# althonos/pyfastani

Hardware: AMD Instinct MI355X
Metric: genome-pair ANI/sec (5 Mb bacterial, 3 kb frags) (higher is better)
Workload: dtype u32

## Files before the change

### pyfastani_amd/csrc/fa_map.hip.h

```cpp
#pragma once

#include "fa_common.h"
#include "fa_compact.hip.h"
#include "fa_mapstream.h"
#include "fa_policy.h"
#include "fa_sketch.hip.h"
#include "fa_sketch_fast.hip.h"

namespace fa {



constexpr int MAP_THREADS = 256;
constexpr uint32_t SEED_PAD = 0xFFFFFFFFu;

__device__ inline void block_bitonic_sort(uint32_t *a, uint32_t n32) {
  for (uint32_t size = 2; size <= n32; size <<= 1) {
    for (uint32_t stride = size >> 1; stride > 0; stride >>= 1) {
      __syncthreads();
      for (uint32_t t = threadIdx.x; t < n32 / 2; t += blockDim.x) {
        uint32_t lo = 2 * t - (t & (stride - 1));
        uint32_t hi = lo + stride;
        bool up = (lo & size) == 0;
        uint32_t x = a[lo], y = a[hi];
// ... 1441 lines not shown
    atomicAdd(&a.counters[CNT_OFF_FAST], 1u);
  }
  __threadfence_block();
  __syncthreads();
  const uint32_t nl = sh_cnt, base = sh_base;
  for (uint32_t q = tid; q < nl; q += NT) {
    const uint32_t li = base + q;
    a.l_frag[li] = f; a.l_rfirst[li] = S_rfirst[q]; a.l_rpart[li] = S_rpart[q]; a.l_rlast[li] = S_rlast[q];
  }
  l1_locus_fields<NT>(a.ix, len, nl, S_rfirst, S_rpart, S_rlast, a.l_seq + base, a.l_start + base, a.l_end + base);
  __threadfence_block();
  __syncthreads();
  if (wv == 0) l1_number_groups(a.ix, nl, a.l_seq + base, a.l_group + base, base);
}

struct TieKey {
  uint32_t flip, add;
  __host__ __device__ uint32_t encode(uint32_t x) const { return (x + add) ^ flip; }
  __host__ __device__ uint32_t decode(uint32_t low) const { return (low ^ flip) - add; }
  static TieKey of(int largest) { TieKey t; t.flip = largest ? 0u : 0xFFFFFFFFu; t.add = largest ? 1u : 0u; return t; }
};

struct L2Args {
  IndexView ix;
  const uint32_t *q_hash;
  const int32_t *q_size;
  const int32_t *l_frag, *l_seq, *l_start, *l_end, *l_group, *l_rfirst, *l_rlast, *l_rpart;
  int32_t frag_len;
  int32_t *l_beg, *l_end0, *l_last;
  int32_t *l_ndrop;
  uint32_t *l_nev;
  uint32_t *l_ioff;
  unsigned long long *pinfo;
  uint64_t items_cap;
  int32_t l_cap;
  void *items;
  int32_t *l_shared, *l_pos;
  const int32_t *pass_lut;
  unsigned long long *group_best;
  const uint32_t *counters;
  LociRegions loci;
  int32_t qcap, cmw;
  int32_t cnt_slots;
  int32_t lanes;
  int32_t ev_stage;
  unsigned long long *rec_total;
  unsigned long long *ev_region, *rec_region;
  uint64_t region_cap;
  uint32_t n_regions;
  uint8_t *l_redo;
  uint32_t *redo_count;
  const uint32_t *f_loci_lo, *f_loci_n;
  const int32_t *frag_order;
  unsigned long long *stamp;
  uint32_t *scan_hist, *scan_cursor;
  uint32_t *scan_order;
  int32_t scan_class_div;
  int32_t slide_end;
  TieKey tie;
};

constexpr int L2_THREADS = 64;
constexpr int EV_THREADS = 256;
constexpr int SCAN_CLASSES = 32;
__device__ __forceinline__ uint32_t scan_class(uint32_t nev, int32_t div) {
  return (uint32_t)(SCAN_CLASSES - 1) - min((uint32_t)(SCAN_CLASSES - 1), nev / (uint32_t)div);
}

template <typename T> struct EvBits;
template <> struct EvBits<uint16_t> { static constexpr int RANK = EV_RANK16; };
template <> struct EvBits<uint32_t> { static constexpr int RANK = 24; };
constexpr int EV_DM = 0, EV_DW = 2, EV_DROP = 5, EV_SLOT = 6;
template <typename T> constexpr uint32_t ev_noeval() { return 1u << (8 * sizeof(T) - 1); }
template <typename T> constexpr uint32_t ev_slot_mask() { return ((1u << EvBits<T>::RANK) - 1u) << EV_SLOT; }
static_assert(EV_SLOT + EvBits<uint16_t>::RANK == 15 && EV_SLOT + EvBits<uint32_t>::RANK <= 31, "event fields overlap");

#ifndef FA_EV_WAVES
#define FA_EV_WAVES 8
#endif
constexpr int EV_WAVES_PER_SIMD = FA_EV_WAVES;
constexpr int EV_SENTINELS = 4;
#ifndef FA_EV_RPL
#define FA_EV_RPL 4
#endif
constexpr int EV_RPL = FA_EV_RPL;
static_assert(EV_RPL >= 1 && EV_RPL <= 4, "the last trip of a phase is dispatched on 1..4 records per lane");
__host__ __device__ inline size_t ev_sketch_bytes(int cnt_slots) { return ((size_t)(cnt_slots - 1 + EV_SENTINELS) * 4 + 15) / 16 * 16; }

constexpr int EV_OCC_BITS = 10, EV_SUB_BITS = 5;
template <typename T, bool PACKED>
__global__ __launch_bounds__(EV_THREADS, EV_WAVES_PER_SIMD) void k_l2_events(L2Args a) {
  extern __shared__ __align__(16) unsigned char lds[];
  stage_stamp(a.stamp);
  uint32_t *Q = (uint32_t *)lds;
  constexpr int QT_BITS = EV_OCC_BITS + EV_SUB_BITS;
  constexpr int OCC_N = (1 << EV_OCC_BITS) + 1;
  constexpr uint32_t SUB_MASK = (1u << EV_SUB_BITS) - 1u;
  static_assert(EV_SUB_BITS == 5, "one 32-bit occupancy word per bucket");
  __shared__ __align__(8) unsigned char rank_table[OCC_N * 4 + (OCC_N + 1) * 2];
  uint32_t *const OCC = (uint32_t *)rank_table;
  uint16_t *const R0 = (uint16_t *)(rank_table + OCC_N * 4);
  const int f = a.frag_order ? a.frag_order[blockIdx.x] : (int)blockIdx.x;
  if (f < 0) return;
  const uint32_t l_lo = a.f_loci_lo[f], l_n = a.f_loci_n[f];
  if (l_n == 0) return;
  const int s = a.q_size[f];
  const int lane = threadIdx.x & 63, wv = threadIdx.x >> 6;
  if (a.counters[CNT_LOCI_OVF] || s > a.cnt_slots - 1) return;
  for (int i = threadIdx.x; i < s + EV_SENTINELS; i += EV_THREADS) Q[i] = i < s ? a.q_hash[(size_t)f * a.qcap + i] : 0xFFFFFFFFu;
  for (int b = threadIdx.x; b < OCC_N; b += EV_THREADS) { OCC[b] = 0u; R0[b] = (uint16_t)s; }
  __shared__ uint32_t sh_wave[EV_THREADS / 64];
  __shared__ uint32_t sh_run, sh_base, sh_ok;
  __shared__ unsigned long long sh_records;
  __shared__ uint32_t sh_class[SCAN_CLASSES];
  if (threadIdx.x == 0) { sh_run = 0; sh_records = 0; }
  if (threadIdx.x < SCAN_CLASSES) sh_class[threadIdx.x] = 0;
  __syncthreads();
  const int32_t *wpos = a.ix.rec_wpos;
  for (uint32_t c0 = 0; c0 < l_n; c0 += EV_THREADS) {
    const uint32_t l = l_lo + c0 + threadIdx.x;
    uint32_t nev = 0, records = 0;
    if (c0 + threadIdx.x < l_n) {
      const int lo = a.ix.contig_rec[a.l_seq[l]];
      const int rfirst = a.l_rfirst[l], target = a.l_start[l], rpart = a.l_rpart[l];
      int last = a.ix.rec_fwd[a.l_rlast[l]];
      if (a.slide_end) {
        const int tgt = wpos[a.l_rlast[l]] + a.frag_len;
        int u = last, v = min(a.ix.contig_rec[a.l_seq[l] + 1], last + (a.frag_len - a.cmw));
        while (u < v) { int mid = u + ((v - u) >> 1); if (wpos[mid] < tgt) u = mid + 1; else v = mid; }
        last = u;
      }
      int x = max(lo, rfirst - a.frag_len), y = rfirst;
      if (rpart >= 0) {
        y = min(rfirst, a.ix.rec_bwd[rpart] + 1);
        x = max(x, y - (a.frag_len - a.cmw + 1));
      }
      while (x < y) { int mid = x + ((y - x) >> 1); if (wpos[mid] < target) x = mid + 1; else y = mid; }
      const int beg = x;
      const int end0 = a.ix.rec_fwd[beg];
      const int ndrop = last > end0 ? a.ix.rec_bwd[last - 1] - beg : 0;
      a.l_beg[l] = beg; a.l_end0[l] = end0; a.l_last[l] = last; a.l_ndrop[l] = ndrop;
      nev = (uint32_t)((((end0 - beg + 7) & ~7) + (last - end0) + ndrop + 7) & ~7);
      records = (uint32_t)(last - beg);
      a.l_nev[l] = nev;
      if (a.scan_class_div) atomicAdd(&sh_class[scan_class(nev, a.scan_class_div)], 1u);
    }
    uint32_t incl = nev;
    for (int d = 1; d < 64; d <<= 1) { uint32_t o = __shfl_up(incl, d); if (lane >= d) incl += o; }
    if (lane == 63) sh_wave[wv] = incl;
    uint32_t rsum = records;
    for (int d = 32; d > 0; d >>= 1) rsum += __shfl_down(rsum, d);
    if (lane == 0) atomicAdd(&sh_records, (unsigned long long)rsum);
    __syncthreads();
    uint32_t off = sh_run + incl - nev;
    for (int q = 0; q < wv; q++) off += sh_wave[q];
// ... 175 lines not shown
        const int rem = hi - t0;
        auto tail = [&](auto rpl_tag) __attribute__((always_inline)) { issue(rpl_tag, t, FIRST, t0, hi); work(rpl_tag, first_tag, store, t, cur, t0, hi); };
        if (rem > 64 * 3) tail(std::integral_constant<int, (EV_RPL >= 4 ? 4 : EV_RPL)>());
        else if (rem > 64 * 2) tail(std::integral_constant<int, (EV_RPL >= 3 ? 3 : EV_RPL)>());
        else if (rem > 64) tail(std::integral_constant<int, (EV_RPL >= 2 ? 2 : EV_RPL)>());
        else if (rem > 0) tail(std::integral_constant<int, 1>());
      };
      phase(std::true_type(), cur.beg, cur.end0);
      phase(std::false_type(), cur.end0, cur.last);
    };
    if (st.staged) run([&](uint32_t pos, uint32_t v) __attribute__((always_inline)) { *(lds_out_t)(uintptr_t)(obase + pos * (uint32_t)sizeof(T)) = (T)v; });
    else { T *gout = st.gout; run([&](uint32_t pos, uint32_t v) __attribute__((always_inline)) { gout[pos] = (T)v; }); }
    end_locus(st);
  }
}

template <typename T, typename ST, int LNT, bool BASE0>
struct Slide {
  typedef __attribute__((address_space(3))) ST *lds_ptr;
  static constexpr int STB = (int)sizeof(ST);
  static constexpr int SBITS = 8 * STB;
  static constexpr int RB = EvBits<T>::RANK;
  int lbase, LNB, s;
  int rl, g, shared, best, beg, opt_s, opt_e;
  uint32_t overflow;

  static __device__ __forceinline__ uint32_t ld(int addr) { return (uint32_t)*(lds_ptr)(uintptr_t)(uint32_t)addr; }
  static __device__ __forceinline__ void sto(int addr, uint32_t v) { *(lds_ptr)(uintptr_t)(uint32_t)addr = (ST)v; }

  __device__ __forceinline__ void init(ST *st, int lane, int lanes, int sketch, int beg0) {
    lbase = (int)(uint32_t)(uintptr_t)(lds_ptr)st + lane * STB;
    LNB = (LNT ? LNT : lanes) * STB;
    s = sketch;
    rl = lbase; g = 0; shared = 0; best = -1; beg = opt_s = opt_e = beg0; overflow = 0;
  }
  static constexpr uint32_t EMPTY = 2u;
  __device__ __forceinline__ void clear() { for (int i = 0; i <= s + 1; i++) sto(i * LNB + lbase, EMPTY); }
  template <int SH> __device__ __forceinline__ int slot_addr(uint32_t word) const {
    if constexpr (LNT == 64) {
      const uint32_t row = (SH ? word >> SH : word) & ev_slot_mask<T>();
      if constexpr (BASE0) return (int)((STB == 1 ? row : row * STB) | (uint32_t)lbase);
      else return (int)(STB == 1 ? row : row * STB) + lbase;
    } else {
      return (int)__builtin_amdgcn_ubfe(word, SH + EV_SLOT, RB) * LNB + lbase;
    }
  }
  template <int SH> __device__ __forceinline__ void fill(uint32_t word) {
    const int dM = __builtin_amdgcn_sbfe(word, SH + EV_DM, 2), dW = __builtin_amdgcn_sbfe(word, SH + EV_DW, 2);
    const int addr = slot_addr<SH>(word);
    const uint32_t nv = (ld(addr) + (uint32_t)(dW << 1)) ^ ((uint32_t)dM & 1u);
    overflow |= nv;
    sto(addr, nv);
  }
  __device__ __forceinline__ void read_pivot() {
    int rstar = s, F = s, acc = 0, m_acc = 0;
    bool hit = false;
    for (int r = 0; r < s; r++) {
      const uint32_t v = ld((r + 1) * LNB + lbase);
      const int c = (int)(v >> 1) - 1, mt = (int)(v & 1u);
      const bool now = !hit && r + acc + c >= s;
      rstar = now ? r : rstar;
      F = now ? r + acc : F;
      shared = now ? m_acc : shared;
      hit = hit || now;
      acc += c; m_acc += mt;
    }
    F = hit ? F : s + acc;
    shared = hit ? shared : m_acc;
    g = F - s;
    rl = rstar * LNB + lbase;
    best = shared;
  }
  template <int SH> __device__ __forceinline__ void step(uint32_t word) {
    const int dM = __builtin_amdgcn_sbfe(word, SH + EV_DM, 2), dW = __builtin_amdgcn_sbfe(word, SH + EV_DW, 2);
    const int drp = (int)__builtin_amdgcn_ubfe(word, SH + EV_DROP, 1);
    const int addr = slot_addr<SH>(word);
    const int addrb = rl + drp * LNB;
    const uint32_t v = ld(addr), vb0 = ld(addrb);
    const uint32_t nv = (v + (uint32_t)(dW << 1)) ^ ((uint32_t)dM & 1u);
    overflow |= nv;
    sto(addr, nv);
    const bool below = addr <= rl;
    const int dWb = below ? dW : 0;
    shared += below ? dM : 0;
    g += dWb;
    const uint32_t vb = (addrb == addr) ? nv : vb0;
    const int c1 = (int)(vb >> 1), mbm = __builtin_amdgcn_sbfe(vb, 0, 1);
    const bool up = ((dW & (g + c1 - 1)) < 0);
    const bool down = dWb > 0 && g > 0;
    const int delta = up ? 1 : (down ? -1 : 0);
    g += __mul24(delta, c1);
    shared += delta & mbm;
    rl += __mul24(delta, LNB);
    beg += drp;
    const int sh_e = (int)((uint32_t)shared | ((word << ((32 - SH - 8 * (int)sizeof(T)) & 31)) & 0x80000000u));
    const bool gt = sh_e > best, ge = sh_e >= best;
    best = max(best, sh_e);
    opt_s = gt ? beg : opt_s;
    opt_e = ge ? beg : opt_e;
  }
};

__global__ __launch_bounds__(256) void k_l2_order(L2Args a) {
  __shared__ uint32_t sh_cnt[SCAN_CLASSES], sh_at[SCAN_CLASSES];
  const uint32_t r = blockIdx.x & (a.loci.n - 1u), off = (blockIdx.x / a.loci.n) * 256u + threadIdx.x;
  if (a.counters[CNT_LOCI_OVF] || a.pinfo[PI_FLAGS]) return;
  const uint32_t live = min(a.loci.count[r], 1u << a.loci.shift);
  if ((blockIdx.x / a.loci.n) * 256u >= live) return;
  if (threadIdx.x < SCAN_CLASSES) sh_cnt[threadIdx.x] = 0;
  __syncthreads();
  const uint32_t l = (r << a.loci.shift) + off;
  uint32_t c = 0, rank = 0;
  if (off < live) { c = scan_class(a.l_nev[l], a.scan_class_div); rank = atomicAdd(&sh_cnt[c], 1u); }
  __syncthreads();
  if (threadIdx.x < SCAN_CLASSES) {
    uint32_t before = 0;
    for (uint32_t q = 0; q < threadIdx.x; q++) before += a.scan_hist[r * SCAN_CLASSES + q];
    sh_at[threadIdx.x] = before + (sh_cnt[threadIdx.x] ? atomicAdd(&a.scan_cursor[r * SCAN_CLASSES + threadIdx.x], sh_cnt[threadIdx.x]) : 0u);
  }
  __syncthreads();
  if (off < live) a.scan_order[(r << a.loci.shift) + min(sh_at[c] + rank, (1u << a.loci.shift) - 1u)] = l;
}

template <typename T, typename ST, int LNT>
__global__ __launch_bounds__(L2_THREADS) void k_l2_scan(L2Args a) {
  extern __shared__ __align__(16) unsigned char lds[];
  constexpr bool REDO = sizeof(ST) > 1;
  const int LN = LNT ? LNT : a.lanes;
  ST *st = (ST *)lds;
  const int lane = threadIdx.x;
  if (lane >= LN) return;
  const uint32_t region = blockIdx.x & (a.loci.n - 1u), off = (blockIdx.x / a.loci.n) * (uint32_t)LN + (uint32_t)lane;
  if (a.counters[CNT_LOCI_OVF] || off >= (1u << a.loci.shift) || off >= a.loci.count[region]) return;
  if (a.scan_order && a.pinfo[PI_FLAGS]) return;
  const uint32_t l = a.scan_order ? a.scan_order[(region << a.loci.shift) + off] : (region << a.loci.shift) + off;
  if (REDO) { if (!a.l_redo[l]) return; }
  else a.l_redo[l] = 0;
  const int s = a.q_size[a.l_frag[l]];
  if (s + 1 > a.cnt_slots) return;
  const int beg0 = a.l_beg[l];
  const uint32_t nev = a.l_nev[l];
  constexpr int PER = 16 / sizeof(T);
  const uint4 *ev = (const uint4 *)((const T *)a.items + a.l_ioff[l]);
  Slide<T, ST, LNT, true> sl;
  sl.init(st, lane, LN, s, beg0);
  sl.clear();
  if (sl.lbase != lane * (int)sizeof(ST)) __builtin_trap();

  const uint32_t ngroups = nev / PER;
  const uint32_t fill_groups = min(ngroups, (uint32_t)((((a.l_end0[l] - beg0) + 7) & ~7) / PER));
  auto word_of = [](const uint4 &g, int q) __attribute__((always_inline)) {
    constexpr int WPE = (int)sizeof(T);
    return (q * WPE / 4 == 0) ? g.x : (q * WPE / 4 == 1) ? g.y : (q * WPE / 4 == 2) ? g.z : g.w;
  };
  uint4 cur = ngroups ? ev[0] : make_uint4(0, 0, 0, 0);
  for (uint32_t g = 0; g < fill_groups; g++) {
    const uint4 nxt = (g + 1 < ngroups) ? ev[g + 1] : make_uint4(0, 0, 0, 0);
#pragma unroll
    for (int q = 0; q < PER; q++) {
      if (sizeof(T) == 2 && (q & 1)) sl.template fill<16>(word_of(cur, q)); else sl.template fill<0>(word_of(cur, q));
    }
    cur = nxt;
  }
  sl.read_pivot();
  if (!fill_groups) sl.best = -1;
  for (uint32_t g = fill_groups; g < ngroups; g++) {
    const uint4 nxt = (g + 1 < ngroups) ? ev[g + 1] : make_uint4(0, 0, 0, 0);
#pragma unroll
    for (int q = 0; q < PER; q++) {
      if (sizeof(T) == 2 && (q & 1)) sl.template step<16>(word_of(cur, q)); else sl.template step<0>(word_of(cur, q));
    }
    cur = nxt;
  }
  if (sl.overflow >> Slide<T, ST, LNT, true>::SBITS) {
    if (!REDO) { a.l_redo[l] = 1; atomicAdd(a.redo_count, 1u); return; }
  }
  a.l_shared[l] = sl.best < 0 ? 0 : sl.best;
  a.l_pos[l] = (a.ix.rec_wpos[sl.opt_s] + a.ix.rec_wpos[sl.opt_e]) / 2;
  if (sl.best >= a.pass_lut[s]) {
    unsigned long long key = ((unsigned long long)(uint32_t)sl.best << 32) | (unsigned long long)a.tie.encode(l);
    atomicMax(&a.group_best[a.l_group[l]], key);
  }
}

struct CgiArgs {
  IndexView ix;
  const unsigned long long *group_best;
  const uint32_t *counters;
  const int32_t *l_frag, *l_seq, *l_pos;
  const int32_t *q_size;
  const float *ident_lut;
  const int32_t *frag_query;
  const int32_t *frag_qseq;
  unsigned long long *bins;
  int32_t bin_len;
  int32_t query_base;
  uint32_t group_bound;
  int32_t wide_launched;
  unsigned long long *stamp;
  TieKey tie;
};

struct MapWinner { int32_t ref_seq_id, ref_start_pos, conserved, sketch_size; };
static_assert(sizeof(MapWinner) == 16, "a winner entry is written with one 16-byte store");

__device__ __forceinline__ bool cgi_survivor(const CgiArgs &a, uint32_t g, size_t &idx, unsigned long long &key, MapWinner &win) {
  if (a.counters[CNT_LOCI_OVF] || g >= a.group_bound) return false;
  if (a.counters[CNT_WIDE] && !a.wide_launched) return false;
  unsigned long long best = a.group_best[g];
  if (best == 0) return false;
  uint32_t l = a.tie.decode((uint32_t)(best & 0xFFFFFFFFu));
  int shared = (int)(best >> 32);
  int f = a.l_frag[l];
  int s = a.q_size[f];
  float ident = a.ident_lut[(size_t)s * (size_t)(s + 1) / 2 + shared];
  int seq = a.l_seq[l];
  int pos = a.l_pos[l];
// ... 257 lines not shown
```

### pyfastani_amd/csrc/fa_policy.h

```cpp
#pragma once

#include <algorithm>
#include <cstddef>
#include <cstdint>
#include <vector>

#include "fa_error.h"

namespace fa {

constexpr int L1_STAGE = 128;
constexpr uint32_t L1_SMALL_HITS = 16u * 256u, L1_MID_HITS = 16u * 512u - 256u;
constexpr int L1_INPLACE_MAX = 32;
constexpr int LOCI_REGIONS = 64;
constexpr int EV_REGIONS = 64;
constexpr int EV_RANK16 = 9;

constexpr uint32_t SPEC_SMAX = 1, SPEC_SCRATCH = 2, SPEC_LOCI = 4, SPEC_EVENTS = 8, SPEC_QFUSE = 16;
constexpr uint32_t SPEC_LAST = SPEC_QFUSE;
constexpr uint32_t SPEC_VOID = SPEC_SMAX | SPEC_SCRATCH | SPEC_LOCI | SPEC_EVENTS | SPEC_QFUSE;
static_assert(SPEC_VOID == 2 * SPEC_LAST - 1, "every SPEC_* flag voids the part (k_l2_order / k_l2_scan rely on it)");

enum StatSlot : int {
  STAT_SMAX = 0,
  STAT_SMALL, STAT_MID, STAT_TINY,
};
enum TotalSlot : int {
  TOT_SEEDS = 0,
  TOT_MAX_FRAG,
  TOT_SCRATCH,
  TOT_RECORDS,
};
enum CounterSlot : int {
  CNT_MERGED = 0,
  CNT_OFF_FAST,
  CNT_LOCI_OVF,
  CNT_WIDE,
  CNT_ROWS_DONE,
  CNT_L1_SORTED, CNT_L1_MERGED,
};
enum PinfoSlot : int {
  PI_EVENTS = 0,
  PI_FLAGS,
};

struct PassStatus {
  int32_t stats[4];
  int32_t total_rows, pad0;
  int64_t total_maps;
  uint64_t totals[4];
  uint32_t counters[8];
  unsigned long long pinfo[4];
  unsigned long long ev_region[EV_REGIONS], rec_region[EV_REGIONS];
  uint32_t loci_region[LOCI_REGIONS];
  unsigned long long dbg[16];
  unsigned long long stamp[6];
  uint32_t seq, pad1;
};
static_assert(offsetof(PassStatus, stamp) % 16 == 0, "k_clear zeroes whole 16-byte words: the cleared prefix of the status block must end on one");

// ... 18 lines not shown
  Spec s;
  s.init = true;
  s.smax = smax;
  s.seed_slots = 4096;
  s.scratch_words = 0;
  s.l_cap = l_cap;
  s.items_cap = items_cap;
  s.part_frags = part_frags;
  return s;
}

inline void spec_merge(Spec &ms, const Spec &sp) {
  ms.smax = std::max(ms.smax, sp.smax);
  ms.seed_slots = sp.seed_slots;
  ms.scratch_words = std::max(ms.scratch_words, sp.scratch_words);
  ms.items_cap = std::max(ms.items_cap, sp.items_cap);
  ms.l_cap = std::max(ms.l_cap, sp.l_cap);
  ms.part_frags = std::min(ms.part_frags, sp.part_frags);
  ms.redo = ms.redo || sp.redo;
  ms.l1_small_share = sp.l1_small_share; ms.l1_mid_share = sp.l1_mid_share; ms.l1_tiny_share = sp.l1_tiny_share;
  ms.l1_prefilter = ms.l1_prefilter || sp.l1_prefilter; ms.l1_no_small = ms.l1_no_small || sp.l1_no_small;
  ms.l2_loci_last = sp.l2_loci_last;
  ms.smax_misses = std::max(ms.smax_misses, sp.smax_misses);
}

inline void fuse_overflowed(Spec &ms) {
  ms.fuse_penalty = ms.fuse_penalty ? std::min(64, ms.fuse_penalty * 2) : 1;
  ms.fuse_skip = ms.fuse_penalty - 1;
}
inline void fuse_accepted(Spec &ms, bool fused, bool skipped) {
  if (fused) ms.fuse_penalty = 0;
  else if (skipped && ms.fuse_skip > 0) ms.fuse_skip--;
}

inline int floor_log2(int v) {
  int l = 0;
  while (((int64_t)2 << l) <= v) l++;
  return l;
}

inline uint32_t ev_regions_for(int64_t F) {
  uint32_t n = 1;
  while (n < (uint32_t)EV_REGIONS && (int64_t)n * 16 <= F) n <<= 1;
  return n;
}

inline uint32_t lds_seed_cap_max(int smax) {
  const int64_t room = 160 * 1024 - 2048 - (int64_t)L1_STAGE * 6 * 4 - std::max<int64_t>(((int64_t)smax + 2) * 8, 1024 * 10) - 64;
  return (uint32_t)std::max<int64_t>(256, room / 4 / 256 * 256);
}

inline bool knob_or(int knob, bool dflt) { return knob < 0 ? dflt : knob != 0; }

inline uint32_t build_frag_order(const int64_t *genome_frag_lo, int32_t g0, int64_t f0, int64_t f1, std::vector<int32_t> &out) {
  const int64_t F = f1 - f0;
  out.clear();
  int32_t q = g0;
  while (genome_frag_lo[q + 1] <= f0) q++;
  if (genome_frag_lo[q + 1] >= f1) {
    if (F < 64) return 0;
    const int64_t run = (F + 7) / 8;
    out.assign((size_t)run * 8, -1);
    for (int64_t i = 0; i < F; i++) out[(size_t)((i % run) * 8 + i / run)] = (int32_t)i;
    return (uint32_t)out.size();
  }
  std::vector<int32_t> off((size_t)F);
  int32_t max_off = 0;
  for (int64_t i = 0, qq = q; i < F; i++) {
    while (genome_frag_lo[qq + 1] <= f0 + i) qq++;
    off[(size_t)i] = (int32_t)(f0 + i - genome_frag_lo[qq]);
    max_off = std::max(max_off, off[(size_t)i]);
  }
  if (max_off + 1 < 8) return 0;
  std::vector<int32_t> start((size_t)max_off + 2, 0);
  for (int64_t i = 0; i < F; i++) start[(size_t)off[(size_t)i] + 1]++;
  for (int32_t p = 0; p <= max_off; p++) start[(size_t)p + 1] += start[(size_t)p];
  std::vector<int32_t> sorted((size_t)F), fill(start.begin(), start.end() - 1);
  for (int64_t i = 0; i < F; i++) sorted[(size_t)fill[(size_t)off[(size_t)i]]++] = (int32_t)i;
  size_t len[8] = {0};
  std::vector<uint8_t> xcd_of((size_t)max_off + 1);
  for (int32_t p = 0; p <= max_off; p++) {
    int x = 0;
    for (int i = 1; i < 8; i++) if (len[i] < len[x]) x = i;
    xcd_of[(size_t)p] = (uint8_t)x;
    len[x] += (size_t)(start[(size_t)p + 1] - start[(size_t)p]);
  }
  const size_t longest = *std::max_element(len, len + 8);
  if ((double)longest * 8.0 > 1.15 * (double)F) return 0;
  out.assign(longest * 8, -1);
  size_t at[8] = {0};
  for (int32_t p = 0; p <= max_off; p++) {
    const size_t x = xcd_of[(size_t)p];
    for (int32_t i = start[(size_t)p]; i < start[(size_t)p + 1]; i++) out[(at[x]++) * 8 + x] = sorted[(size_t)i];
  }
  return (uint32_t)out.size();
}

struct Forms {
  int n_l1 = 0, l1_threads[3] = {0, 0, 0};
  bool prefilter = false, scan_sorted = false, wide = false, fused = false, ordered = false, redo = false;
  int smax = 0;
  uint32_t seed_slots = 0;
  bool small_class() const { return n_l1 > 1 && l1_threads[0] == 256; }
};

struct L1Class { int nt; uint32_t slots, n_lo, n_hi; };
struct L1Plan {
  L1Class c[3];
  int n = 0;
  bool prefilter = false;
  uint32_t need = 0;
  uint32_t seed_slots() const { return c[n - 1].slots; }
};
struct L1Knobs { int prefilter = -1; float thin_small = -1.0f, thin_mid = 0.05f; };

inline L1Plan plan_l1(const Spec &sp, int64_t records, const L1Knobs &k) {
// ... 126 lines not shown
```

### pyfastani_amd/csrc/fa_query.hip.h

```cpp
#pragma once

#include <algorithm>
#include <chrono>
#include <cstddef>
#include <deque>
#include <initializer_list>
#include <memory>
#include <mutex>
#include <string>
#include <vector>

#include "fa_batch.hip.h"
#include "fa_common.h"
#include "fa_index.hip.h"
#include "fa_lease.h"
#include "fa_mapstream.h"
#include "fa_policy.h"

using namespace fa;

static PublishArgs publish_args(PassStatus *dev, PassStatus *host_mapped, uint32_t seq, const fa_cgi_row *rows_dev, fa_cgi_row *rows_host, int64_t cap) {
  PublishArgs p;
  p.status_dev = (uint32_t *)dev; p.status_host = (uint32_t *)host_mapped;
  p.words = (int32_t)(offsetof(PassStatus, seq) / 4); p.seq_word = p.words; p.seq = seq;
// ... 176 lines not shown
    ea.n_bins = (int64_t)NQ * m.total_bins; ea.total_bins = std::max(m.total_bins, 1); ea.query_id_base = g0; ea.n_chunks = map_chunks;
    ea.chunk_count = w.map_chunk_count.p; ea.chunk_off = w.map_chunk_off.p;
    ea.maps = nullptr; ea.tie = TieKey::of(w.rules.cgi_ties);
    if (map_chunks) hipLaunchKernelGGL(k_map_count, dim3(map_chunks), dim3(256), 0, st, ea);
    hipLaunchKernelGGL(k_chunk_scan, dim3(1), dim3(1024), 0, st, ea.chunk_count, ea.chunk_off, ea.n_chunks, &w.status.p->total_maps);
    if (!map_chunks || maps.count_only) return;
    int64_t hi = maps.stage;
    ea.maps = w.map_stage.dev[0];
    if (maps.dev) { ea.maps = maps.dev + maps.base; hi = std::max<int64_t>(0, maps.cap - maps.base); }
    hipLaunchKernelGGL(k_map_write, dim3(map_chunks), dim3(256), 0, st, ea, (int64_t)0, hi);
  }
  void stream_maps(MapSink &sink) {
    MapStage &sg = w.map_stage;
    const int64_t total = nmaps, n_win = map_windows(total, sink.stage);
    auto issue = [&](int64_t wi) {
      const MapWindow win = map_window(total, sink.stage, wi);
      const int s = (int)(wi & 1);
      if (wi > 0) {
        MapEmitArgs ea = map_args;
        ea.maps = sg.dev[s];
        hipLaunchKernelGGL(k_map_write, dim3(map_chunks), dim3(256), 0, st, ea, win.lo, win.hi);
      }
      FA_HIP(hipMemcpyAsync(sg.pin[s], sg.dev[s], (size_t)(win.hi - win.lo) * sizeof(fa_hit_mapping), hipMemcpyDeviceToHost, st));
      FA_HIP(hipEventRecord(sg.ev[s], st));
    };
    if (n_win) issue(0);
    for (int64_t wi = 0; wi < n_win; wi++) {
      if (wi + 1 < n_win) issue(wi + 1);
      const MapWindow win = map_window(total, sink.stage, wi);
      FA_HIP(hipEventSynchronize(sg.ev[wi & 1]));
      if (sink.host) {
        memcpy(sink.host + sink.base + win.lo, sg.pin[wi & 1], (size_t)(win.hi - win.lo) * sizeof(fa_hit_mapping));
        continue;
      }
      const int rc = sink.fn(sink.user, sg.pin[wi & 1], win.hi - win.lo);
      if (rc != 0) {
        (void)hipStreamSynchronize(st);
        throw Error(FA_ERR_INVALID, "the mapping sink ended the call (it returned " + std::to_string(rc) + ")");
      }
    }
  }
  struct Part {
    const Spec &sp;
    const int64_t f0, f1, F;
    const int t0, ntiles;
    const int smax;
    const int64_t l_cap;
    L1Plan l1;
    bool scan_sorted = false;
    bool wide = false;
    LociRegions loci{nullptr, 1, 0};
    const int32_t *frag_order = nullptr;
    uint32_t order_len = 0;
    int32_t *d_stats = nullptr;
    uint64_t *d_totals = nullptr;
    uint32_t *d_counters = nullptr;
    unsigned long long *d_pinfo = nullptr;
    Part(QueryPass &q, Run &r)
        : sp(r.sp), f0(r.f0), f1(r.f1), F(r.f1 - r.f0), t0(q.g.frag_tile_lo[r.f0]),
          ntiles(q.g.frag_tile_lo[r.f1] - q.g.frag_tile_lo[r.f0]), smax(r.sp.smax),
          l_cap(std::max<int64_t>(r.sp.l_cap, (int64_t)std::min<uint32_t>(LOCI_REGIONS, ev_regions_for(r.f1 - r.f0)))) {}
  };

  void launch_part(Run &r) {
    Part p(*this, r);
    const Spec &sp = p.sp;
    const int64_t f0 = p.f0, F = p.F;
    w.last_F = 0; w.last_loci = 0;
    ev_packed = m.events_packed();
    const int ntiles = p.ntiles;
    w.sk.reserve((size_t)std::max(ntiles, 1));
    w.q_hash.ensure((size_t)F * qcap); w.q_off.ensure((size_t)F * qcap); w.q_cnt.ensure((size_t)F * qcap);
    w.q_size.ensure((size_t)F); w.n_seeds.ensure((size_t)F); w.ovf_off.ensure((size_t)F);
    w.f_loci_lo.ensure((size_t)F); w.f_loci_n.ensure((size_t)F);
    w.status.ensure(1);
    if (!w.h_status) {
      w.pin_status.ensure(sizeof(PassStatus), hipHostMallocMapped | hipHostMallocCoherent);
      w.h_status = (PassStatus *)w.pin_status.p;
      memset(w.h_status, 0, sizeof(PassStatus));
    }
    p.d_stats = w.status.p->stats; p.d_totals = w.status.p->totals; p.d_counters = w.status.p->counters; p.d_pinfo = w.status.p->pinfo;
    const int smax = p.smax;
    const int64_t l_cap = p.l_cap;
    {
      const L1Knobs knobs{(int)knob::l1_prefilter(), (float)knob::l1_thin_small(), (float)knob::l1_thin_mid()};
      p.l1 = plan_l1(sp, m.N, knobs);
      if (knob::debug_l1()) fprintf(stderr, "k_l1 classes: need=%u tiny=%.3f small=%.3f mid=%.3f prefilter=%d -> %d launch(es)\n", p.l1.need, sp.l1_tiny_share, sp.l1_small_share, sp.l1_mid_share, (int)p.l1.prefilter, p.l1.n);
    }
    w.l_frag.ensure((size_t)l_cap); w.l_seq.ensure((size_t)l_cap); w.l_start.ensure((size_t)l_cap); w.l_end.ensure((size_t)l_cap + 4);
    w.l_rfirst.ensure((size_t)l_cap); w.l_rlast.ensure((size_t)l_cap + 4); w.l_rpart.ensure((size_t)l_cap);
    w.l_group.ensure((size_t)l_cap); w.l_shared.ensure((size_t)l_cap); w.l_pos.ensure((size_t)l_cap);
    w.group_best.ensure((size_t)l_cap + 2);
    w.l_beg.ensure((size_t)l_cap); w.l_end0.ensure((size_t)l_cap); w.l_last.ensure((size_t)l_cap); w.l_ndrop.ensure((size_t)l_cap);
    w.l_nev.ensure((size_t)l_cap); w.l_ioff.ensure((size_t)l_cap); w.l_redo.ensure((size_t)l_cap + 4);
    p.scan_sorted = scan_sorted(sp, (int)knob::l2_scan_order());
    w.scan_hist.ensure((size_t)2 * LOCI_REGIONS * SCAN_CLASSES);
    if (p.scan_sorted) w.scan_order.ensure((size_t)l_cap + 64);
    w.ovf_buf.ensure((size_t)sp.scratch_words + 4);
    p.loci.count = w.status.p->loci_region;
    p.loci.n = std::min<uint32_t>(LOCI_REGIONS, ev_regions_for(F));
    p.loci.shift = (uint32_t)floor_log2((int)std::max<int64_t>(1, l_cap / p.loci.n));
    w.loci_n = p.loci.n; w.loci_shift = p.loci.shift;
    p.wide = wide_events(smax);
    w.items.ensure(((size_t)sp.items_cap + 8) * (p.wide ? 4 : 2));
    w.forms = Forms();
    w.forms.n_l1 = p.l1.n;
    for (int c = 0; c < p.l1.n; c++) w.forms.l1_threads[c] = p.l1.c[c].nt;
    w.forms.prefilter = p.l1.prefilter; w.forms.scan_sorted = p.scan_sorted; w.forms.wide = p.wide; w.forms.redo = sp.redo;
    w.forms.smax = smax; w.forms.seed_slots = p.l1.seed_slots();

    launch_sketch_stage(r, p);
    prepare_order(p);
    launch_l1_stage(p);
    launch_l2_stage(r, p);
    launch_cgi_stage_and_hand_over(r, p);
  }

  void prepare_order(Part &p) {
    if (!frag_order_gate(knob::frag_order() != 0, knob::frag_order_one() != 0, NQ, p.F)) return;
    if (w.order_batch != g.serial || w.order_f0 != p.f0 || w.order_f1 != p.f1) {
      std::vector<int32_t> ord;
      w.order_len = build_frag_order(g.genome_frag_lo.data(), g0, p.f0, p.f1, ord);
      if (w.order_len) {
        w.pin_order.ensure(ord.size() * sizeof(int32_t));
        memcpy(w.pin_order.p, ord.data(), ord.size() * sizeof(int32_t));
        w.frag_order.ensure(ord.size());
        FA_HIP(hipMemcpyAsync(w.frag_order.p, w.pin_order.p, ord.size() * sizeof(int32_t), hipMemcpyHostToDevice, st));
      }
      w.order_batch = g.serial; w.order_f0 = p.f0; w.order_f1 = p.f1;
    }
    if (w.order_len) { p.frag_order = w.frag_order.p; p.order_len = w.order_len; }
  }

  void launch_sketch_stage(Run &r, Part &p) {
    const Spec &sp = p.sp;
    const int64_t f0 = p.f0, F = p.F;
    const int64_t l_cap = p.l_cap;
    const int t0 = p.t0, ntiles = p.ntiles;
    {
      ClearList cl;
      cl.add(w.status.p, offsetof(PassStatus, stamp));
      cl.a.stamp = &w.status.p->stamp[0];
      cl.add(w.l_end.p, (size_t)l_cap * sizeof(int32_t)); cl.add(w.l_rlast.p, (size_t)l_cap * sizeof(int32_t));
      cl.add(w.group_best.p, (size_t)l_cap * sizeof(unsigned long long));
      if (p.scan_sorted) cl.add(w.scan_hist.p, (size_t)2 * LOCI_REGIONS * SCAN_CLASSES * sizeof(uint32_t));
      if (!bins_cleared) {
        cl.add(w.bins.p, (size_t)NQ * std::max(m.total_bins, 1) * sizeof(unsigned long long));
        if (maps.on) cl.add(w.winners.p, (size_t)NQ * std::max(m.total_bins, 1) * sizeof(MapWinner));
        bins_cleared = true;
      }
      QuerySketchArgs a;
      a.frag_tile_lo = g.d_frag_tile_lo + f0;
      a.tile_count = w.sk.tile_count.p; a.stage_hash = w.sk.stage_hash.p; a.stage_wpos = w.sk.stage_wpos.p;
      a.tile_base = t0;
      a.q_hash = w.q_hash.p; a.q_size = w.q_size.p; a.qcap = qcap;
      a.ix = ix; a.q_off = w.q_off.p; a.q_cnt = w.q_cnt.p; a.n_seeds = w.n_seeds.p;
      a.sort_cap = (int32_t)(qs_lds / 4);
      a.rec_cap = (int)std::max(0.0, std::min((double)QF_CAP, knob::qf_cap()));
      a.exc_tiles = 0;
      const bool fused = launch_sketch_tiles(m.P, g.store, g.tiles + t0, ntiles, w.sk.stage_hash.p, w.sk.stage_wpos.p, w.sk.tile_count.p, st, &cl.a,
                                             (sp.fuse_off || r.forced_unfused) ? nullptr : &a, F);
      r.fused = fused;
      if (!fused) launch_lds(k_query_sketch, dim3((unsigned)F), dim3(MAP_THREADS), qs_lds, st, a);
    }
    debug_sync(st, "sketch");
  }

  void launch_l1_stage(Part &p) {
    const Spec &sp = p.sp;
    const int64_t F = p.F;
    const int smax = p.smax;
    const int64_t l_cap = p.l_cap;
// ... 31 lines not shown
      }
      auto go = [&](auto nt_tag, const L1Class &c, bool fold) {
        constexpr int NTT = decltype(nt_tag)::value;
        const size_t lds = l1_lds_bytes(c.slots, smax, NTT);
        FA_REQUIRE(lds + 1024 <= 160 * 1024, FA_ERR_UNSUPPORTED, "query sketch too large for the LDS tables of the L1 kernel");
        if (knob::debug_l1()) fprintf(stderr, "k_l1<%d>: F=%lld hits %u..%u seed_slots=%u smax=%d lds=%zu\n", NTT, (long long)F, c.n_lo, c.n_hi, c.slots, smax, lds);
        L1Args b = a;
        b.lds_seed_cap = c.slots; b.n_lo = c.n_lo; b.n_hi = c.n_hi; b.fold_totals = fold ? 1 : 0;
        constexpr uint32_t E_MAX = NTT == 256 ? 16u : (uint32_t)L1_INPLACE_MAX;
        FA_REQUIRE(c.slots <= E_MAX * (uint32_t)NTT, FA_ERR_INTERNAL, "more seed slots than a workgroup of the L1 kernel merges");
        const auto kernel = c.slots <= 16u * (uint32_t)NTT ? k_l1<NTT, 16> : k_l1<NTT, (int)E_MAX>;
        launch_lds(kernel, dim3(l1_grid + (fold ? 1u : 0u)), dim3(NTT), lds, st, b);
      };
      for (int c = 0; c < p.l1.n; c++) {
        const bool fold = fold_totals && c == 0;
        if (p.l1.c[c].nt >= 512) go(std::integral_constant<int, 512>(), p.l1.c[c], fold);
        else go(std::integral_constant<int, 256>(), p.l1.c[c], fold);
      }
    }
    debug_sync(st, "l1");
  }

  void launch_l2_stage(Run &r, Part &p) {
    const Spec &sp = p.sp;
    const int64_t F = p.F;
    const int smax = p.smax;
    const int64_t l_cap = p.l_cap;
    const bool wide = p.wide;
    {
      if (m.stage_events) FA_HIP(hipEventRecord(w.ev[0], st));
      L2Args a;
      a.stamp = &w.status.p->stamp[2];
      a.ix = ix; a.q_hash = w.q_hash.p; a.q_size = w.q_size.p;
      a.l_frag = w.l_frag.p; a.l_seq = w.l_seq.p; a.l_start = w.l_start.p; a.l_end = w.l_end.p; a.l_group = w.l_group.p;
      a.l_rfirst = w.l_rfirst.p; a.l_rlast = w.l_rlast.p; a.l_rpart = w.l_rpart.p; a.frag_len = m.P.fragment_length;
      a.l_beg = w.l_beg.p; a.l_end0 = w.l_end0.p; a.l_last = w.l_last.p; a.l_nev = w.l_nev.p; a.l_ioff = w.l_ioff.p; a.l_ndrop = w.l_ndrop.p;
      a.items = w.items.p; a.items_cap = sp.items_cap; a.pinfo = p.d_pinfo; a.l_cap = (int32_t)l_cap;
      a.l_shared = w.l_shared.p; a.l_pos = w.l_pos.p; a.pass_lut = w.lut_pass; a.group_best = w.group_best.p;
      a.counters = p.d_counters; a.loci = p.loci; a.qcap = qcap; a.cmw = m.cmw;
      a.cnt_slots = smax + 1;
      a.rec_total = (unsigned long long *)&p.d_totals[TOT_RECORDS];
      a.ev_region = w.status.p->ev_region; a.rec_region = w.status.p->rec_region;
      a.n_regions = ev_regions_for(F);
      a.region_cap = (sp.items_cap / a.n_regions) & ~7ULL;
      a.l_redo = w.l_redo.p;
      a.redo_count = &p.d_counters[CNT_WIDE];
      const L2Lds lds(m.P, smax, wide);
      a.scan_class_div = p.scan_sorted ? lds.scan_class_div : 0;
      a.scan_hist = w.scan_hist.p; a.scan_cursor = w.scan_hist.p + LOCI_REGIONS * SCAN_CLASSES;
      a.scan_order = p.scan_sorted ? w.scan_order.p : nullptr;
      a.slide_end = w.rules.slide_end; a.tie = TieKey::of(w.rules.cgi_ties);
      a.f_loci_lo = w.f_loci_lo.p; a.f_loci_n = w.f_loci_n.p;
      a.frag_order = p.frag_order;
      const uint32_t ev_grid = p.frag_order ? p.order_len : (uint32_t)F;
      if (p.frag_order) r.ordered = true;
      a.ev_stage = lds.ev_stage;
      const size_t ev_lds = lds.events;
      FA_REQUIRE(ev_lds <= 150 * 1024, FA_ERR_UNSUPPORTED, "query sketch too large for the LDS-staged event kernel");
      auto pick_lanes = [&](int bytes) {
        int ln = L2_THREADS;
        while (ln > 1 && lds.scan(ln, bytes) > 144 * 1024) ln >>= 1;
        FA_REQUIRE(lds.scan(ln, bytes) <= 160 * 1024, FA_ERR_UNSUPPORTED, "query sketch too large for the LDS-resident L2 state");
        return ln;
      };
      const int lanes8 = pick_lanes(1), lanes16 = pick_lanes(2);
      const size_t lds8 = lds.scan(lanes8, 1), lds16 = lds.scan(lanes16, 2);
      auto scan_grid = [&](int lanes) { return (unsigned)(p.loci.n * (uint32_t)ceil_div((int64_t)1 << p.loci.shift, lanes)); };
      auto launch = [&](auto ev_kernel, auto scan8, auto scan8_rt, auto scan16, auto scan16_rt) {
        launch_lds(ev_kernel, dim3(ev_grid), dim3(EV_THREADS), ev_lds, st, a);
        debug_sync(st, "l2 events");
        if (p.scan_sorted)
          hipLaunchKernelGGL(k_l2_order, dim3((unsigned)(p.loci.n * (uint32_t)ceil_div((int64_t)1 << p.loci.shift, 256))), dim3(256), 0, st, a);
        a.lanes = lanes8;
        launch_lds(lanes8 == L2_THREADS ? scan8 : scan8_rt, dim3(scan_grid(lanes8)), dim3(L2_THREADS), lds8, st, a);
        if (!sp.redo) return;
        a.lanes = lanes16;
        launch_lds(lanes16 == L2_THREADS ? scan16 : scan16_rt, dim3(scan_grid(lanes16)), dim3(L2_THREADS), lds16, st, a);
      };
      const bool pk = ev_packed;
      if (wide) launch(pk ? k_l2_events<uint32_t, true> : k_l2_events<uint32_t, false>, k_l2_scan<uint32_t, uint8_t, 64>, k_l2_scan<uint32_t, uint8_t, 0>, k_l2_scan<uint32_t, uint16_t, 64>, k_l2_scan<uint32_t, uint16_t, 0>);
      else launch(pk ? k_l2_events<uint16_t, true> : k_l2_events<uint16_t, false>, k_l2_scan<uint16_t, uint8_t, 64>, k_l2_scan<uint16_t, uint8_t, 0>, k_l2_scan<uint16_t, uint16_t, 64>, k_l2_scan<uint16_t, uint16_t, 0>);
    }
    debug_sync(st, "l2 scan");
    if (m.stage_events) FA_HIP(hipEventRecord(w.ev[1], st));
  }

  void launch_cgi_stage_and_hand_over(Run &r, Part &p) {
    const Spec &sp = p.sp;
    const int64_t f0 = p.f0;
    const int64_t l_cap = p.l_cap;
    if (npairs > 0) {
      CgiArgs a;
      a.stamp = &w.status.p->stamp[3];
      a.ix = ix; a.group_best = w.group_best.p; a.counters = p.d_counters; a.l_frag = w.l_frag.p; a.l_seq = w.l_seq.p;
      a.l_pos = w.l_pos.p; a.q_size = w.q_size.p; a.ident_lut = w.lut_ident;
      a.frag_query = g.d_frag_query + f0; a.frag_qseq = g.d_frag_qseq + f0; a.bins = w.bins.p;
      a.bin_len = m.P.fragment_length - 20;
      a.query_base = g0;
      a.wide_launched = sp.redo ? 1 : 0;
      a.tie = TieKey::of(w.rules.cgi_ties);
      a.group_bound = p.loci.n << p.loci.shift;
      hipLaunchKernelGGL(k_cgi_bins, dim3(ceil_div(l_cap, 256)), dim3(256), 0, st, a);
      if (maps.on) hipLaunchKernelGGL(k_cgi_winners, dim3(ceil_div(l_cap, 256)), dim3(256), 0, st, a, w.winners.p);
    }
    if (r.with_rows) rows_valid = true;
    hand_over(r.with_rows);
  }
  void hand_over(bool rows) {
// ... 289 lines not shown
```

Baseline: 205,900.

## Compute one-genome fragment order on device and early-exit pivot scan

When all fragments of a part belong to one genome, the event kernel now derives the interleaved fragment order arithmetically from the block index. This replaces building the order table on the host and copying it to the device. The pivot read in the sliding-window state is rewritten to accumulate counts in blocks of eight ranks and exit once every lane in the wavefront has passed the pivot, instead of always walking all s ranks. The trade-off is extra ballot operations, and the shared-count derivation from summed slot values must match the old semantics exactly.

```diff
diff --git a/pyfastani_amd/csrc/fa_map.hip.h b/pyfastani_amd/csrc/fa_map.hip.h
--- a/pyfastani_amd/csrc/fa_map.hip.h
+++ b/pyfastani_amd/csrc/fa_map.hip.h
@@ -1517,6 +1517,7 @@
   uint32_t *redo_count;
   const uint32_t *f_loci_lo, *f_loci_n;
   const int32_t *frag_order;
+  uint32_t one_run, one_frags;
   unsigned long long *stamp;
   uint32_t *scan_hist, *scan_cursor;
   uint32_t *scan_order;
@@ -1565,7 +1566,7 @@
   __shared__ __align__(8) unsigned char rank_table[OCC_N * 4 + (OCC_N + 1) * 2];
   uint32_t *const OCC = (uint32_t *)rank_table;
   uint16_t *const R0 = (uint16_t *)(rank_table + OCC_N * 4);
-  const int f = a.frag_order ? a.frag_order[blockIdx.x] : (int)blockIdx.x;
+  const int f = a.one_run ? one_genome_frag(blockIdx.x, a.one_run, a.one_frags) : a.frag_order ? a.frag_order[blockIdx.x] : (int)blockIdx.x;
   if (f < 0) return;
   const uint32_t l_lo = a.f_loci_lo[f], l_n = a.f_loci_n[f];
   if (l_n == 0) return;
@@ -1847,21 +1848,27 @@
     overflow |= nv;
     sto(addr, nv);
   }
-  __device__ __forceinline__ void read_pivot() {
-    int rstar = s, F = s, acc = 0, m_acc = 0;
-    bool hit = false;
-    for (int r = 0; r < s; r++) {
-      const uint32_t v = ld((r + 1) * LNB + lbase);
-      const int c = (int)(v >> 1) - 1, mt = (int)(v & 1u);
-      const bool now = !hit && r + acc + c >= s;
-      rstar = now ? r : rstar;
-      F = now ? r + acc : F;
-      shared = now ? m_acc : shared;
-      hit = hit || now;
-      acc += c; m_acc += mt;
-    }
-    F = hit ? F : s + acc;
-    shared = hit ? shared : m_acc;
+  __device__ __forceinline__ void read_pivot(int ranks) {
+    int rstar = 0, F = 0, su = 0, addr = LNB + lbase;
+    uint32_t vsum = 0;
+    bool open = true;
+    auto rank = [&](int r) __attribute__((always_inline)) {
+      const uint32_t v = ld(addr);
+      addr += LNB;
+      su += (int)(v >> 1);
+      open = su <= s && r < s;
+      rstar += open ? 1 : 0;
+      F = open ? su : F;
+      vsum += open ? v : 0u;
+    };
+    int r = 0;
+    for (; r + 8 <= ranks; r += 8) {
+#pragma unroll
+      for (int q = 0; q < 8; q++) rank(r + q);
+      if (!__ballot(open)) break;
+    }
+    for (; r < ranks && __ballot(open); r++) rank(r);
+    shared = (int)vsum - 2 * F;
     g = F - s;
     rl = rstar * LNB + lbase;
     best = shared;
@@ -1957,7 +1964,7 @@
     }
     cur = nxt;
   }
-  sl.read_pivot();
+  sl.read_pivot(a.cnt_slots - 1);
   if (!fill_groups) sl.best = -1;
   for (uint32_t g = fill_groups; g < ngroups; g++) {
     const uint4 nxt = (g + 1 < ngroups) ? ev[g + 1] : make_uint4(0, 0, 0, 0);
diff --git a/pyfastani_amd/csrc/fa_policy.h b/pyfastani_amd/csrc/fa_policy.h
--- a/pyfastani_amd/csrc/fa_policy.h
+++ b/pyfastani_amd/csrc/fa_policy.h
@@ -6,6 +6,12 @@
 #include <vector>
 
 #include "fa_error.h"
+
+#if defined(__HIPCC__)
+#define FA_POLICY_FN __host__ __device__ inline
+#else
+#define FA_POLICY_FN inline
+#endif
 
 namespace fa {
 
@@ -130,16 +136,28 @@
 
 inline bool knob_or(int knob, bool dflt) { return knob < 0 ? dflt : knob != 0; }
 
+FA_POLICY_FN uint32_t one_genome_run(int64_t F) { return F < 64 ? 0u : (uint32_t)((F + 7) / 8); }
+FA_POLICY_FN int32_t one_genome_frag(uint32_t b, uint32_t run, uint32_t F) {
+  const uint32_t i = (b & 7u) * run + (b >> 3);
+  return (b >> 3) < run && i < F ? (int32_t)i : -1;
+}
+FA_POLICY_FN int32_t one_genome_frag(uint32_t b, uint32_t F) { return one_genome_frag(b, (F + 7u) / 8u, F); }
+inline bool frag_range_in_one_genome(const int64_t *genome_frag_lo, int32_t g0, int64_t f0, int64_t f1) {
+  int32_t q = g0;
+  while (genome_frag_lo[q + 1] <= f0) q++;
+  return genome_frag_lo[q + 1] >= f1;
+}
+
 inline uint32_t build_frag_order(const int64_t *genome_frag_lo, int32_t g0, int64_t f0, int64_t f1, std::vector<int32_t> &out) {
   const int64_t F = f1 - f0;
   out.clear();
   int32_t q = g0;
   while (genome_frag_lo[q + 1] <= f0) q++;
-  if (genome_frag_lo[q + 1] >= f1) {
-    if (F < 64) return 0;
-    const int64_t run = (F + 7) / 8;
-    out.assign((size_t)run * 8, -1);
-    for (int64_t i = 0; i < F; i++) out[(size_t)((i % run) * 8 + i / run)] = (int32_t)i;
+  if (frag_range_in_one_genome(genome_frag_lo, g0, f0, f1)) {
+    const uint32_t run = one_genome_run(F);
+    if (!run) return 0;
+    out.resize((size_t)run * 8);
+    for (uint32_t b = 0; b < run * 8; b++) out[b] = one_genome_frag(b, run, (uint32_t)F);
     return (uint32_t)out.size();
   }
   std::vector<int32_t> off((size_t)F);
diff --git a/pyfastani_amd/csrc/fa_query.hip.h b/pyfastani_amd/csrc/fa_query.hip.h
--- a/pyfastani_amd/csrc/fa_query.hip.h
+++ b/pyfastani_amd/csrc/fa_query.hip.h
@@ -252,6 +252,7 @@
     LociRegions loci{nullptr, 1, 0};
     const int32_t *frag_order = nullptr;
     uint32_t order_len = 0;
+    uint32_t order_run = 0;
     int32_t *d_stats = nullptr;
     uint64_t *d_totals = nullptr;
     uint32_t *d_counters = nullptr;
@@ -318,6 +319,7 @@
 
   void prepare_order(Part &p) {
     if (!frag_order_gate(knob::frag_order() != 0, knob::frag_order_one() != 0, NQ, p.F)) return;
+    if (frag_range_in_one_genome(g.genome_frag_lo.data(), g0, p.f0, p.f1)) { p.order_run = one_genome_run(p.F); return; }
     if (w.order_batch != g.serial || w.order_f0 != p.f0 || w.order_f1 != p.f1) {
       std::vector<int32_t> ord;
       w.order_len = build_frag_order(g.genome_frag_lo.data(), g0, p.f0, p.f1, ord);
@@ -455,8 +457,9 @@
       a.slide_end = w.rules.slide_end; a.tie = TieKey::of(w.rules.cgi_ties);
       a.f_loci_lo = w.f_loci_lo.p; a.f_loci_n = w.f_loci_n.p;
       a.frag_order = p.frag_order;
-      const uint32_t ev_grid = p.frag_order ? p.order_len : (uint32_t)F;
-      if (p.frag_order) r.ordered = true;
+      a.one_run = p.order_run; a.one_frags = (uint32_t)F;
+      const uint32_t ev_grid = p.order_run ? 8u * p.order_run : p.frag_order ? p.order_len : (uint32_t)F;
+      if (p.frag_order || p.order_run) r.ordered = true;
       a.ev_stage = lds.ev_stage;
       const size_t ev_lds = lds.events;
       FA_REQUIRE(ev_lds <= 150 * 1024, FA_ERR_UNSUPPORTED, "query sketch too large for the LDS-staged event kernel");
```

New measurement: 212,300 (median of 6 runs). 1.03x the previous value.
